# FishYuLi/BalancedGroupSoftmax

Measured on AMD Instinct MI355X. Metric: img/s fwd+bwd R50-FPN+BAGS 1333x800, 512 RoI (BASELINE metric: img/s/GPU fwd+bwd R50-FPN+BAGS 1333x800, 512 RoI; GroupSoftmax us/RoI), higher is better.
Workload: dtype f32 (conv/linear products on the bf16 MFMA from exact 3-way bf16 splits, fp32 accumulate: fp32-faithful)

## Files before the change

balancedgroupsoftmax_amd/backbone.py:

```python
import contextlib

import torch
import torch.nn as nn

from . import functional as BF
from .ops import OFFSET_PITCH, DeformConv
from .registry import BACKBONES, NECKS


def _trainable(*modules):
    return torch.is_grad_enabled() and any(
        p.requires_grad for m in modules if m is not None for p in m.parameters())


def _fold_conv_bn(conv, bn, pad_cin_to=None):
    w = conv.weight
    cbias = getattr(conv, 'bias', None)
    if w.is_cuda:
        ctx = contextlib.nullcontext() if _trainable(conv, bn) else torch.no_grad()
        with ctx:
            if bn is not None:
                return BF.fold_conv_bn(w, cbias, bn.weight, bn.bias, bn.running_mean,
                                       bn.running_var, bn.eps, cin_padded=pad_cin_to)
            return BF.fold_conv_bn(w, cbias, cin_padded=pad_cin_to)
# ... 124 lines not shown
    def _build_fold(self):
        f = dict(c1=_fold_conv_bn(self.conv1, self.bn1), c2=_fold_conv_bn(self.conv2, self.bn2),
                 c3=_fold_conv_bn(self.conv3, self.bn3))
        if self.downsample is not None:
            f['ds'] = _fold_conv_bn(self.downsample[0], self.downsample[1])
        if self.with_dcn:
            ow, ob = _fold_conv_bn(self.conv2_offset, None)
            padc = OFFSET_PITCH - ow.shape[0]
            f['off'] = (torch.nn.functional.pad(ow, (0, 0, 0, 0, 0, 0, 0, padc)).contiguous(),
                        torch.nn.functional.pad(ob, (0, padc)).contiguous())
        return f

    def run_bf16_storage(self, x, f):
        if self.with_dcn:
            raise NotImplementedError('Bottleneck.run_bf16_storage: a dcn block has no bf16-storage kernel '
                                      '(the deformable conv is fp32 only)')
        identity, fk = x, None
        if 'ds' in f:
            if x.is_cuda and BF.shortcut_fork_enabled():
                with BF.forked(x.device) as fk:
                    identity = BF.conv2d_nhwc(x, f['ds'][0], f['ds'][1], stride=self.stride)
            else:
                identity = BF.conv2d_nhwc(x, f['ds'][0], f['ds'][1], stride=self.stride)
        out = BF.conv2d_nhwc(x, f['c1'][0], f['c1'][1], relu=True)
        if self.groups > 1:
            out = BF.grouped_conv3x3_nhwc(out, f['c2'][0], f['c2'][1], self.groups, stride=self.stride,
                                          relu=True)
        else:
            out = BF.conv2d_nhwc(out, f['c2'][0], f['c2'][1], stride=self.stride, pad=1, relu=True)
        if fk is not None:
            fk.join()
        return BF.conv2d_nhwc(out, f['c3'][0], f['c3'][1], relu=True, residual=identity)

    def run(self, x, f):
        if x.dtype == torch.bfloat16:
            return self.run_bf16_storage(x, f)
        tagged = bool(getattr(x, '_bgs_consumers_mask', False))
        fuse = BF.fork_fusion_enabled() and torch.is_grad_enabled() and x.requires_grad
        if tagged and not fuse:
            raise RuntimeError("Bottleneck.run: x is a relu='consumers' block output but fork fusion is off")
        out_relu = 'consumers' if BF.fork_fusion_enabled() else True
        xin = x
        identity = x
        fk = None
        if 'ds' in f and not fuse and x.is_cuda and BF.shortcut_fork_enabled() and \
                not (torch.is_grad_enabled() and any(t.requires_grad for t in f['ds'] if t is not None)):
            with BF.forked(x.device) as fk:
                identity = BF.conv2d_nhwc(x, f['ds'][0], f['ds'][1], stride=self.stride)
        elif 'ds' in f:
            if fuse:
                identity, xin = BF.conv2d_autograd(x, f['ds'][0], f['ds'][1], stride=self.stride,
                                                   mask_input=tagged, passthrough=True)
            else:
                identity = BF.conv2d_autograd(x, f['ds'][0], f['ds'][1], stride=self.stride)
        first_pt = fuse and 'ds' not in f
        first_mask = tagged and 'ds' not in f
        if self.groups > 1 or self.with_dcn:
            out = BF.conv2d_autograd(xin, f['c1'][0], f['c1'][1], relu=True, mask_input=first_mask,
                                     passthrough=first_pt)
            if first_pt:
                out, identity = out
            if self.with_dcn:
                off = BF.conv2d_autograd(out, f['off'][0], f['off'][1], stride=self.stride, pad=1)
                out = BF.deform_conv3x3_nhwc(out, off, f['c2'][0], f['c2'][1], self.dcn_groups,
                                             stride=self.stride, relu=True)
            else:
                out = BF.grouped_conv3x3_nhwc(out, f['c2'][0], f['c2'][1], self.groups,
                                              stride=self.stride, relu=True)
            if fk is not None:
                fk.join()
            return BF.conv2d_autograd(out, f['c3'][0], f['c3'][1], relu=out_relu, residual=identity)
        out = BF.conv2d_autograd(xin, f['c1'][0], f['c1'][1], relu='consumers', mask_input=first_mask,
                                 passthrough=first_pt)
        if first_pt:
            out, identity = out
        if not fuse and BF.fused_c3_eligible(out, f['c2'][0], f['c3'][0], self.stride, identity):
            if fk is not None:
                fk.join()
            return BF.conv3x3_c3_fused_nhwc(out, f['c2'][0], f['c2'][1], f['c3'][0], f['c3'][1], residual=identity,
                                            relu3=True)
        out = BF.conv2d_autograd(out, f['c2'][0], f['c2'][1], stride=self.stride, pad=1,
                                 relu='consumers', mask_input=True)
        if fk is not None:
            fk.join()
        return BF.conv2d_autograd(out, f['c3'][0], f['c3'][1], relu=out_relu, residual=identity,
                                  mask_input=True)


@BACKBONES.register_module
class ResNet(nn.Module):
    arch_settings = {50: (3, 4, 6, 3), 101: (3, 4, 23, 3), 152: (3, 8, 36, 3)}

    def __init__(self, depth, num_stages=4, strides=(1, 2, 2, 2), dilations=(1, 1, 1, 1),
                 out_indices=(0, 1, 2, 3), style='pytorch', frozen_stages=-1, conv_cfg=None,
                 norm_cfg=dict(type='BN', requires_grad=True), norm_eval=True, dcn=None,
                 stage_with_dcn=(False, False, False, False), gcb=None,
                 stage_with_gcb=(False, False, False, False), gen_attention=None,
                 stage_with_gen_attention=((), (), (), ()), with_cp=False,
                 zero_init_residual=True, groups=1, base_width=4):
        super().__init__()
        if depth not in self.arch_settings:
            raise KeyError('invalid depth {} for resnet (bottleneck depths only)'.format(depth))
        if dcn:
            raise NotImplementedError('dcn (deformable convolution, gs_htc_dconv_* config) has no '
                                      'kernel in this build')
        if style != 'pytorch' or tuple(dilations) != (1, 1, 1, 1) or gcb or gen_attention:
            raise NotImplementedError('only the plain pytorch-style trunk of the BAGS configs')
        if norm_cfg.get('type', 'BN') != 'BN' or not norm_eval:
            raise NotImplementedError('BatchNorm in eval mode only (norm_eval=True is what every '
                                      'BAGS config uses); it is folded into the convs')
        self.depth, self.num_stages = depth, num_stages
# ... 46 lines not shown
        elif pretrained is not None:
            raise TypeError('pretrained must be a str or None')
        for m in self.modules():
            if isinstance(m, nn.Conv2d):
                nn.init.kaiming_normal_(m.weight, mode='fan_out', nonlinearity='relu')
            elif isinstance(m, nn.BatchNorm2d):
                nn.init.constant_(m.weight, 1)
                nn.init.constant_(m.bias, 0)
        for m in self.modules():
            if isinstance(m, Bottleneck):
                nn.init.constant_(m.bn3.weight, 0)
                if hasattr(m, 'conv2_offset'):
                    nn.init.constant_(m.conv2_offset.weight, 0)
                    nn.init.constant_(m.conv2_offset.bias, 0)

    def _build_stem(self):
        return _fold_conv_bn(self.conv1, self.bn1, pad_cin_to=4)

    @staticmethod
    def to_nhwc4(img):
        if img.is_cuda and not (torch.is_grad_enabled() and img.requires_grad):
            return BF.nchw_to_nhwc4(img)
        x = img.float().permute(0, 2, 3, 1)
        return torch.nn.functional.pad(x, (0, 4 - x.shape[3])).contiguous()

    def forward(self, img):
        return self.forward_partial(img, -1, len(self.res_layers) - 1)[1]

    def forward_partial(self, x, first, last, outs=()):
        outs = list(outs)
        if first < 0:
            x = self._forward_stem(x)
            first = 0
        for i in range(first, last + 1):
            for blk in getattr(self, self.res_layers[i]):
                x = blk.run(x, blk.folded())
            if i in self.out_indices:
                outs.append(BF.relu_gate(x))
        return x, tuple(outs)

    def _forward_stem(self, img):
        stem = self._cache.get((self.conv1, self.bn1), self._build_stem)
        frozen_stem = not (torch.is_grad_enabled() and (img.requires_grad or stem[0].requires_grad or
                                                        stem[1].requires_grad))
        if img.is_cuda and frozen_stem and img.shape[1] == 3 and tuple(stem[0].shape[:3]) == (64, 7, 7) \
                and BF.stem_fused_enabled():
            ws = self._stem_split.get((self.conv1, self.bn1),
                                      lambda: BF.stem_fused_split_weights(stem[0].detach()))
            x = BF.stem_fused(img, ws, stem[1].detach())
        else:
            x = self.to_nhwc4(img)
            x = BF.conv2d_autograd(x, stem[0], stem[1], stride=2, pad=3, relu=True)
            storage = (BF.bf16_storage_active() and not x.requires_grad and
                       not _trainable(*[getattr(self, n) for n in self.res_layers]))
            x = BF.maxpool3x3s2_nhwc(x, out_dtype=torch.bfloat16 if storage else torch.float32)
        return x

    def train(self, mode=True):
        super().train(mode)
        self._freeze_stages()
        if mode and self.norm_eval:
            for m in self.modules():
                if isinstance(m, nn.BatchNorm2d):
                    m.eval()
        return self


@BACKBONES.register_module
class ResNeXt(ResNet):
# ... 75 lines not shown
```

balancedgroupsoftmax_amd/capi.py:

```python
import ctypes
import os

_PKG = os.path.dirname(os.path.abspath(__file__))

c_i64p = ctypes.c_void_p
c_f32p = ctypes.c_void_p
c_ptr = ctypes.c_void_p

BGS_OK = 0
BGS_MAX_BINS = 16


class BgsLibraryError(RuntimeError):
    pass


class BgsCallError(RuntimeError):
    def __init__(self, fn, code, text):
        super().__init__('%s failed with code %d: %s' % (fn, code, text))
        self.code = code


SIGNATURES = {
    'bgs_version': (ctypes.c_int, []),
# ... 42 lines not shown
                            + [c_ptr]),
    'bgs_conv2d_workspace_bytes': (ctypes.c_size_t, [ctypes.c_longlong, ctypes.c_int]),
    'bgs_conv2d_nhwc_f32_ws': (ctypes.c_int, [c_f32p, c_f32p, c_f32p, c_f32p, c_f32p]
                               + [ctypes.c_int] * 11 + [c_ptr, ctypes.c_size_t, c_ptr]),
    'bgs_conv2d_dgrad_nhwc_f32_ws': (ctypes.c_int, [c_f32p, c_f32p, c_f32p, c_f32p, c_f32p]
                                     + [ctypes.c_int] * 10 + [c_ptr, ctypes.c_size_t, c_ptr]),
    'bgs_conv2d_dgrad_nhwc_f32': (ctypes.c_int, [c_f32p, c_f32p, c_f32p, c_f32p, c_f32p]
                                  + [ctypes.c_int] * 10 + [c_ptr]),
    'bgs_conv2d_wgrad_workspace_bytes': (ctypes.c_size_t, [ctypes.c_int] * 9),
    'bgs_conv2d_wgrad_nhwc_f32': (ctypes.c_int, [c_f32p, c_f32p, c_f32p, c_f32p]
                                  + [ctypes.c_int] * 10 + [c_ptr, c_ptr]),
    'bgs_fold_conv_bn_fwd': (ctypes.c_int, [c_f32p] * 6 + [ctypes.c_float] + [ctypes.c_int] * 5
                             + [c_f32p, c_f32p, c_ptr]),
    'bgs_fold_conv_bn_bwd': (ctypes.c_int, [c_f32p] * 7 + [ctypes.c_float] + [ctypes.c_int] * 5
                             + [c_f32p] * 4 + [c_ptr]),
    'bgs_conv2d_wgrad_bfx_workspace_bytes': (ctypes.c_size_t, [ctypes.c_int] * 9),
    'bgs_conv2d_wgrad_nhwc_f32_bfx': (ctypes.c_int, [c_f32p, c_f32p, c_f32p, c_f32p]
                                      + [ctypes.c_int] * 11 + [c_ptr, c_ptr]),
    'bgs_conv2d_wgrad_bfx_enable': (None, [ctypes.c_int]),
    'bgs_conv3x3_halo_nhwc_f32': (ctypes.c_int, [c_f32p, c_f32p, c_f32p, c_f32p] + [ctypes.c_int] * 6
                                  + [c_ptr]),
    'bgs_conv_bfx_weight_bytes': (ctypes.c_size_t, [ctypes.c_int, ctypes.c_int]),
    'bgs_conv_bfx_split_weights': (ctypes.c_int, [c_f32p, c_ptr, ctypes.c_int, ctypes.c_int, c_ptr]),
    'bgs_conv_dgrad_parity_enable': (None, [ctypes.c_int]),
    'bgs_conv_bfx_split_weights_dgrad': (ctypes.c_int, [c_f32p, c_ptr] + [ctypes.c_int] * 4 + [c_ptr]),
    'bgs_conv_bfx_workspace_bytes': (ctypes.c_size_t, [ctypes.c_longlong, ctypes.c_int, ctypes.c_int]),
    'bgs_conv2d_nhwc_f32_bfx_ws': (ctypes.c_int, [c_f32p, c_ptr, c_f32p, c_f32p, c_f32p]
                                   + [ctypes.c_int] * 12 + [c_ptr, ctypes.c_size_t, c_ptr]),
    'bgs_conv2d_dgrad_nhwc_f32_bfx_ws': (ctypes.c_int, [c_f32p, c_ptr, c_f32p, c_f32p, c_f32p]
                                         + [ctypes.c_int] * 11 + [c_ptr, ctypes.c_size_t, c_ptr]),
    'bgs_conv3x3_halo_bfx_workspace_bytes': (ctypes.c_size_t, [ctypes.c_int] * 5),
    'bgs_conv3x3_c3_fused_nhwc_f32_bfx': (ctypes.c_int, [c_f32p, c_ptr, c_f32p, c_ptr, c_f32p, c_f32p, c_f32p]
                                          + [ctypes.c_int] * 6 + [c_ptr]),
    'bgs_conv3x3_halo_nhwc_f32_bfx': (ctypes.c_int, [c_f32p, c_ptr, c_f32p, c_f32p]
                                      + [ctypes.c_int] * 7 + [c_ptr, ctypes.c_size_t, c_ptr]),
    'bgs_conv3x3_halo_nhwc_f32_bfx_ex': (ctypes.c_int, [c_f32p, c_ptr, c_f32p, c_f32p, c_f32p]
                                         + [ctypes.c_int] * 7 + [c_ptr, ctypes.c_size_t, c_ptr]),
    'bgs_conv3x3_planes_head_nhwc_f32_bfx': (ctypes.c_int, [c_f32p, c_ptr, c_f32p, c_ptr, c_f32p, c_f32p]
                                             + [ctypes.c_int] * 7 + [c_ptr]),
    'bgs_conv3x3_planes_head_eligible': (ctypes.c_int, [ctypes.c_int] * 6),
    'bgs_gs_loss_tuning': (None, [ctypes.c_int]),
    'bgs_gs_head_fold': (None, [ctypes.c_int]),
    'bgs_gs_loss_wavepriv_min_rows': (None, [ctypes.c_int]),
    'bgs_gs_merge_tuning': (None, [ctypes.c_int, ctypes.c_int]),
    'bgs_conv_bfx_wide_tuning': (None, [ctypes.c_int] * 3),
    'bgs_conv_bfx_wide_last_launch': (ctypes.c_int, []),
    'bgs_conv1x1_planes_enable': (None, [ctypes.c_int]),
    'bgs_conv1x1_planes_last_launch': (ctypes.c_int, []),
    'bgs_conv3x3_planes_enable': (None, [ctypes.c_int]),
    'bgs_conv3x3_planes_last_launch': (ctypes.c_int, []),
    'bgs_conv1x1_bres_enable': (None, [ctypes.c_int]),
    'bgs_conv1x1_bres_last_launch': (ctypes.c_int, []),
    'bgs_launch_census': (ctypes.c_int, [ctypes.c_int, ctypes.c_int]),
    'bgs_conv_bfx_tuning': (None, [ctypes.c_int] * 2),
    'bgs_conv_bfx_last_launch': (ctypes.c_int, [c_ptr, c_ptr]),
    'bgs_conv_tuning': (None, [ctypes.c_int] * 4),
    'bgs_conv_last_launch': (ctypes.c_int, [c_ptr, c_ptr, c_ptr, c_ptr]),
    'bgs_conv3x3_halo_bfx_tuning': (None, [ctypes.c_int] * 2),
    'bgs_conv3x3_halo_bfx_last_launch': (ctypes.c_int, [c_ptr, c_ptr]),
    'bgs_conv3x3_halo_bfx_last_wide': (ctypes.c_int, [c_ptr, c_ptr]),
    'bgs_conv3x3_halo_bfx_wide': (ctypes.c_int, [ctypes.c_int]),
    'bgs_grouped_conv3x3_nhwc_f32': (ctypes.c_int, [c_f32p, c_f32p, c_f32p, c_f32p] + [ctypes.c_int] * 7
                                     + [c_ptr]),
    'bgs_grouped_conv3x3_nhwc_bf16ops': (ctypes.c_int, [c_f32p, c_f32p, c_f32p, c_f32p] + [ctypes.c_int] * 7
                                         + [c_ptr]),
    'bgs_grouped_conv3x3_dgrad_nhwc_f32': (ctypes.c_int, [c_f32p, c_f32p, c_f32p] + [ctypes.c_int] * 6
# ... 225 lines not shown
```

balancedgroupsoftmax_amd/csrc/bottleneck_tail_planes.hip:

```cpp
#include <stdlib.h>

#include "conv_args.h"
#include "bfx_split.h"

using namespace bgs_conv;

namespace {

typedef __bf16 bf16x2 __attribute__((ext_vector_type(2)));
typedef __bf16 bf16x8 __attribute__((ext_vector_type(8)));
typedef unsigned u32x2 __attribute__((ext_vector_type(2)));
typedef unsigned u32x4 __attribute__((ext_vector_type(4)));

__device__ __forceinline__ unsigned pk_bf16(float a, float b) {
  const bf16x2 h = __builtin_convertvector(f32x2{a, b}, bf16x2);
  return __builtin_bit_cast(unsigned, h);
}

__device__ __forceinline__ void split3p(const f32x4 v, u32x2& hi, u32x2& mid, u32x2& lo) {
  hi = u32x2{pk_bf16(v[0], v[1]), pk_bf16(v[2], v[3])};
  const f32x4 r = {bfx_resid_lo(hi[0], v[0]), bfx_resid_hi(hi[0], v[1]), bfx_resid_lo(hi[1], v[2]),
                   bfx_resid_hi(hi[1], v[3])};
  mid = u32x2{pk_bf16(r[0], r[1]), pk_bf16(r[2], r[3])};
  const f32x4 r2 = {bfx_resid_lo(mid[0], r[0]), bfx_resid_hi(mid[0], r[1]), bfx_resid_lo(mid[1], r[2]),
                    bfx_resid_hi(mid[1], r[3])};
  lo = u32x2{pk_bf16(r2[0], r2[1]), pk_bf16(r2[2], r2[3])};
}

struct TailArgs {
  const float* x;
  const __bf16* ws2;
  const float* bias2;
  const __bf16* ws3;
  const float* bias3;
  const float* res;
  float* y;
  int N, H, W, relu3;
  int tiles_y, tiles_x, tiles, chunk;
};

constexpr int kOob = 0x7f000000;

__global__ __launch_bounds__(kThreads, 3) void bottleneck_tail_planes_kernel(TailArgs g) {
  constexpr int NS = 3, CM = 64, CO3 = 256, KC2 = 36, KC3 = 4;
  constexpr int PW = 10, PS = 12, PSLOTS = PW * PS;
  constexpr int AQ = PW * PW * 16, AQT = (AQ + kThreads - 1) / kThreads;
  constexpr int KS = PSLOTS * 32, PL = 4 * KS;
  constexpr int LDS_BYTES = NS * PL;
  constexpr int LD2 = CM + 4, S2_BYTES = 64 * LD2 * 4;
  constexpr int Y_OFF = 18 * 1024;
  constexpr int P3_CH = 64 * 32, P3_PL = KC3 * P3_CH;
  constexpr int LD4 = CO3 + 8;
  static_assert(S2_BYTES <= Y_OFF && Y_OFF + NS * P3_PL <= LDS_BYTES && 32 * LD4 * 4 <= LDS_BYTES, "overlays");
  __shared__ __attribute__((aligned(1024))) unsigned char lds[LDS_BYTES];

  const int tid = threadIdx.x, lane = tid & 63;
  const int wave = bgs::uniform(tid >> 6);
  const int wm = wave >> 1, wn = wave & 1;
  const int frow = lane & 31, fk = lane >> 5;
  const int vtile = (int)((blockIdx.x & 7) * g.chunk + (blockIdx.x >> 3));
  if (vtile >= g.tiles) return;
  const int per_img = g.tiles_y * g.tiles_x;
  const int n = vtile / per_img, trem = vtile - n * per_img;
  const int ty = trem / g.tiles_x, tx = trem - ty * g.tiles_x;
  const int h0 = ty * 8 - 1, w0 = tx * 8 - 1;

  const __amdgpu_buffer_rsrc_t x_rsrc = __builtin_amdgcn_make_buffer_rsrc(
      const_cast<float*>(g.x), 0, (int)((size_t)g.N * g.H * g.W * CM * 4), 0x00020000);
  f32x4 ra[AQT];
  int a_dst[AQT];
#pragma unroll
  for (int i = 0; i < AQT; ++i) {
    const int q = tid + kThreads * i;
    const bool use = q < AQ;
    const int pix = use ? q >> 4 : 0, kq = q & 15;
    const int ppy = pix / PW, ppx = pix - ppy * PW;
    const int hi = h0 + ppy, wi = w0 + ppx;
    const bool in = use && hi >= 0 && hi < g.H && wi >= 0 && wi < g.W;
    const int off = in ? (((n * g.H + hi) * g.W + wi) * CM + kq * 4) * 4 : kOob;
    ra[i] = __builtin_bit_cast(f32x4, __builtin_amdgcn_raw_buffer_load_b128(x_rsrc, off, 0, 0));
    const int quad = kq & 3;
// ... 112 lines not shown
#pragma unroll
  for (int kc = 0; kc < KC3; ++kc) {
    if (kc + 1 < KC3) {
      if (kc & 1) load_b3(kc + 1, f3a);
      else load_b3(kc + 1, f3b);
    }
    __builtin_amdgcn_sched_barrier(0);
    const bf16x8 (&fb3)[NS][2] = (kc & 1) ? f3b : f3a;
    bf16x8 fa3[NS][2];
#pragma unroll
    for (int s = 0; s < NS; ++s)
#pragma unroll
      for (int a = 0; a < 2; ++a) fa3[s][a] = *reinterpret_cast<const bf16x8*>(lds + a3_frag[a] + kc * P3_CH + s * P3_PL);
#pragma unroll
    for (int tt = NS - 1; tt >= 0; --tt)
#pragma unroll
      for (int i = 0; i <= tt; ++i)
#pragma unroll
        for (int a = 0; a < 2; ++a)
#pragma unroll
          for (int b = 0; b < 2; ++b)
            acc3[a][b] = __builtin_amdgcn_mfma_f32_32x32x16_bf16(fa3[i][a], fb3[tt - i][b], acc3[a][b], 0, 0, 0);
    __builtin_amdgcn_sched_barrier(0);
  }
  __syncthreads();

  const int e4 = (tid & 63) * 4, er0 = tid >> 6;
  f32x4 bias3 = {0.f, 0.f, 0.f, 0.f};
  if (g.bias3) bias3 = *reinterpret_cast<const f32x4*>(g.bias3 + e4);
  const int out_bytes = (int)((size_t)g.N * g.H * g.W * CO3 * 4);
  const __amdgpu_buffer_rsrc_t res_rsrc = __builtin_amdgcn_make_buffer_rsrc(
      const_cast<float*>(g.res ? g.res : g.x), 0, g.res ? out_bytes : 0, 0x00020000);
  const __amdgpu_buffer_rsrc_t y_rsrc = __builtin_amdgcn_make_buffer_rsrc(g.y, 0, out_bytes, 0x00020000);
#pragma unroll
  for (int a = 0; a < 2; ++a) {
    f32x4 rs[8];
#pragma unroll
    for (int ps = 0; ps < 8; ++ps) {
      const int m = a * 32 + er0 + ps * 4;
      const int ho = min(ty * 8 + (m >> 3), g.H - 1), wo = min(tx * 8 + (m & 7), g.W - 1);
      rs[ps] = __builtin_bit_cast(f32x4, __builtin_amdgcn_raw_buffer_load_b128(res_rsrc, (((n * g.H + ho) * g.W + wo) * CO3 + e4) * 4, 0, 0));
    }
#pragma unroll
    for (int b = 0; b < 2; ++b)
#pragma unroll
      for (int r = 0; r < 16; ++r) {
        const int i = (r & 3) + 8 * (r >> 2) + 4 * (lane >> 5);
        scratch[i * LD4 + wave * 64 + b * 32 + (lane & 31)] = acc3[a][b][r];
      }
    __syncthreads();
#pragma unroll
    for (int ps = 0; ps < 8; ++ps) {
      const int i = er0 + ps * 4;
      const int m = a * 32 + i;
      const int ho = ty * 8 + (m >> 3), wo = tx * 8 + (m & 7);
      f32x4 v = *reinterpret_cast<const f32x4*>(scratch + i * LD4 + e4);
      v += bias3;
      v += rs[ps];
      if (g.relu3) {
#pragma unroll
        for (int t = 0; t < 4; ++t) v[t] = fmaxf(v[t], 0.f);
      }
      if (ho < g.H && wo < g.W)
        __builtin_amdgcn_raw_buffer_store_b128(__builtin_bit_cast(u32x4, v), y_rsrc, (((n * g.H + ho) * g.W + wo) * CO3 + e4) * 4, 0, 0);
    }
    __syncthreads();
  }
}

}

int bgs_internal_bottleneck_tail_planes(const float* x, const void* w2split, const float* bias2, const void* w3split,
                                        const float* bias3, const float* residual, float* y, int N, int H, int W,
                                        int relu3, hipStream_t st) {
  const long long lim = kOob;
  if ((long long)N * H * W * 256 * 4 >= lim) return -1;
  TailArgs g;
  g.x = x;
  g.ws2 = reinterpret_cast<const __bf16*>(w2split);
  g.bias2 = bias2;
  g.ws3 = reinterpret_cast<const __bf16*>(w3split);
  g.bias3 = bias3;
  g.res = residual;
  g.y = y;
  g.N = N; g.H = H; g.W = W; g.relu3 = relu3;
  g.tiles_y = (H + 7) / 8;
  g.tiles_x = (W + 7) / 8;
  g.tiles = N * g.tiles_y * g.tiles_x;
  g.chunk = (g.tiles + 7) / 8;
  hipLaunchKernelGGL(bottleneck_tail_planes_kernel, dim3((unsigned)(8 * g.chunk)), dim3(kThreads), 0, st, g);
  return hipGetLastError() == hipSuccess ? BGS_OK : BGS_ERR_LAUNCH;
}
```

balancedgroupsoftmax_amd/functional.py:

```python
import ctypes
import itertools
import os

import torch

from . import capi

_WS = {}


def _workspace(nbytes, device):
    key = (device.index, capi.raw_stream(device))
    buf = _WS.get(key)
    if buf is None or buf.numel() < nbytes:
        buf = torch.empty(max(int(nbytes), 1 << 20), dtype=torch.uint8, device=device)
        _WS[key] = buf
    return buf


def reset_workspaces():
    _WS.clear()


_SIDE = {}
# ... 726 lines not shown
    capi.check('bgs_conv_bfx_split_weights_dgrad', rc)
    if cacheable:
        if key not in _SPLIT_CACHE and len(_SPLIT_CACHE) >= _SPLIT_CACHE_MAX:
            _SPLIT_CACHE.pop(next(iter(_SPLIT_CACHE)))
        _SPLIT_CACHE[key] = (w_krsc._version, (Cout, R, S, Cin), w_krsc, out, CacheFence(w_krsc.device))
    return out


def conv_bfx_tuning(tile=0, splitk=-1, halo_splits=-1, halo_variant=0, halo_geom=-1, halo_flags=0, halo_wide=-1):
    lib = capi.load()
    lib.bgs_conv_bfx_tuning(int(tile), int(splitk))
    lib.bgs_conv3x3_halo_bfx_tuning(int(halo_splits), int(halo_variant) | ((int(halo_geom) + 1) << 16) |
                                    (int(halo_flags) << 20) | ((int(halo_wide) + 1) << 24))


def set_halo_wide(mode):
    return capi.load().bgs_conv3x3_halo_bfx_wide(int(mode))


def conv_bfx_last_launch():
    import ctypes
    lib = capi.load()
    a, c, d, e, f, g = (ctypes.c_int() for _ in range(6))
    lib.bgs_conv_bfx_last_launch(ctypes.byref(a), ctypes.byref(c))
    lib.bgs_conv3x3_halo_bfx_last_launch(ctypes.byref(d), ctypes.byref(e))
    lib.bgs_conv3x3_halo_bfx_last_wide(ctypes.byref(f), ctypes.byref(g))
    return dict(tile=a.value & ~0x400, ring_stages=3 if a.value & 0x400 else 4, splits=c.value,
                halo_nb=d.value & 0xff, halo_variant=(d.value >> 8) & 0xff, halo_geom=d.value >> 16,
                halo_splits=e.value, halo_wide_units=f.value, halo_tail_units=g.value)


CENSUS = dict(bf16_ring8=0, grouped_lds=1, halo_bfx4=2, dma_ring64=3, gs_head_fused=4, conv1x1_bres=5,
              wgrad_bfx=6, roi_bwd_gather=7, bf16s=8, grouped_bf16s=9, bfx_wide=10, gs_scale_grad=11, halo_wide=12, stem_fused=13, fused_c3=14,
              planes_3x3=15, planes_1x1=16, planes_3x3_head=17)


def launch_census(reset=False):
    lib = capi.load()
    out = {k: lib.bgs_launch_census(v, 0) for k, v in CENSUS.items()}
    if reset:
        lib.bgs_launch_census(0, 1)
    return out


def conv_tuning(tile=0, bk=0, splitk=0, noswizzle=0):
    capi.load().bgs_conv_tuning(int(tile), int(bk), int(splitk), int(noswizzle))


def conv_last_launch():
    import ctypes
    a, b, c, d = (ctypes.c_int() for _ in range(4))
    capi.load().bgs_conv_last_launch(ctypes.byref(a), ctypes.byref(b), ctypes.byref(c), ctypes.byref(d))
    return dict(tile=a.value, bk=b.value, up=c.value, splits=d.value)


def _use_halo_bfx(M, Cout):
    env = os.environ.get('BGS_CONV_HALO')
    if env == '1':
        return True
    if env == '0':
        return False
    return M >= 2000


def _use_halo_kernel(M, Cout):
    env = os.environ.get('BGS_CONV_HALO')
    if env == '1':
# ... 11 lines not shown
    _FUSED_C3[0] = bool(on)
    return prev


def fused_c3_eligible(x, w2, w3, stride, residual):
    env = os.environ.get('BGS_FUSED_C3')
    on = _FUSED_C3[0] if env is None else env != '0'
    return (on and _CONV_MATH[0] == 'bf16x6' and x.is_cuda and x.dtype == torch.float32 and stride == 1
            and tuple(w2.shape[:3]) == (64, 3, 3) and w2.shape[3] == 64 and tuple(w3.shape) == (256, 1, 1, 64)
            and x.shape[3] == 64 and _use_halo_bfx(x.shape[0] * x.shape[1] * x.shape[2], 64)
            and x.shape[0] * ((x.shape[1] + 7) // 8) * ((x.shape[2] + 15) // 16) >= 700
            and not (torch.is_grad_enabled() and (x.requires_grad or w2.requires_grad or w3.requires_grad or
                                                  (residual is not None and residual.requires_grad))))


def conv3x3_c3_fused_nhwc(x, w2_krsc, bias2, w3_krsc, bias3, residual=None, relu3=True, out=None):
    _require_cuda(x, w2_krsc, bias2, w3_krsc, bias3, residual)
    lib = capi.load()
    assert x.dtype == torch.float32 and x.is_contiguous() and x.dim() == 4
    N, H, W, Cmid = x.shape
    Cout3 = w3_krsc.shape[0]
    assert tuple(w2_krsc.shape) == (Cmid, 3, 3, Cmid) and tuple(w3_krsc.shape) == (Cout3, 1, 1, Cmid)
    if residual is not None:
        assert tuple(residual.shape) == (N, H, W, Cout3) and residual.is_contiguous() and residual.dtype == torch.float32
    if out is None:
        out = torch.empty((N, H, W, Cout3), dtype=torch.float32, device=x.device)
    w2s = bfx_split_weights(w2_krsc.view(Cmid, 9 * Cmid), cache=True)
    w3s = bfx_split_weights(w3_krsc.view(Cout3, Cmid), cache=True)
    rc = lib.bgs_conv3x3_c3_fused_nhwc_f32_bfx(capi.ptr(x), capi.ptr(w2s), capi.ptr(bias2), capi.ptr(w3s),
                                               capi.ptr(bias3), capi.ptr(residual), capi.ptr(out), N, H, W, Cmid,
                                               Cout3, int(bool(relu3)), capi.current_stream(x.device))
    capi.check('bgs_conv3x3_c3_fused_nhwc_f32_bfx', rc)
    return out


def rpn_head_fusion_eligible(x, w_conv, w_head):
    if os.environ.get('BGS_RPN_HEAD_FUSION', '1') == '0' or _CONV_MATH[0] != 'bf16x6':
        return False
    if not x.is_cuda or x.dtype != torch.float32 or x.dim() != 4 or w_conv.dim() != 4 or w_head.dim() != 4:
        return False
    N, H, W, Cin = x.shape
    if tuple(w_conv.shape[1:]) != (3, 3, Cin) or tuple(w_head.shape[1:]) != (1, 1, w_conv.shape[0]):
        return False
    if not _use_halo_bfx(N * H * W, w_conv.shape[0]):
        return False
    return bool(capi.load().bgs_conv3x3_planes_head_eligible(N, H, W, Cin, w_conv.shape[0], w_head.shape[0]))


def conv3x3_head_fused_nhwc(x, w_krsc, bias, hw_krsc, hbias, relu=True):
    _require_cuda(x, w_krsc, bias, hw_krsc, hbias)
    lib = capi.load()
    assert x.dtype == torch.float32 and x.is_contiguous() and x.dim() == 4
    N, H, W, Cin = x.shape
    Cout, Ch = w_krsc.shape[0], hw_krsc.shape[0]
    assert tuple(w_krsc.shape) == (Cout, 3, 3, Cin) and tuple(hw_krsc.shape) == (Ch, 1, 1, Cout)
    assert w_krsc.is_contiguous() and hw_krsc.is_contiguous()
    ws = bfx_split_weights(w_krsc.view(Cout, 9 * Cin), cache=True)
    hs = bfx_split_weights(hw_krsc.view(Ch, Cout), cache=True)
    out = torch.empty((N, H, W, Ch), dtype=torch.float32, device=x.device)
    rc = lib.bgs_conv3x3_planes_head_nhwc_f32_bfx(capi.ptr(x), capi.ptr(ws), capi.ptr(bias), capi.ptr(hs),
                                                  capi.ptr(hbias), capi.ptr(out), N, H, W, Cin, Cout,
                                                  int(bool(relu)), Ch, capi.current_stream(x.device))
    capi.check('bgs_conv3x3_planes_head_nhwc_f32_bfx', rc)
    return out


# ... 1846 lines not shown
```

include/bgs.h:

```cpp
#ifndef BGS_H_
#define BGS_H_

#include <stddef.h>
#include <stdint.h>

#ifdef __cplusplus
extern "C" {
#endif

#define BGS_OK 0
#define BGS_ERR_INVALID_ARG 1
#define BGS_ERR_UNSUPPORTED 2
#define BGS_ERR_LAUNCH 3

#define BGS_MAX_BINS 16

typedef void* bgs_stream_t;

int bgs_version(void);
const char* bgs_error_string(int code);



int bgs_gs_prepare(const int64_t* labels, const int64_t* label2binlabel,
// ... 88 lines not shown
                         float* dgamma, float* dbeta, bgs_stream_t stream);


int bgs_conv3x3_halo_nhwc_f32(const float* x, const float* w, const float* bias, float* y, int N,
                              int H, int W, int Cin, int Cout, int relu, bgs_stream_t stream);

size_t bgs_conv_bfx_weight_bytes(int rows, int K);
int bgs_conv_bfx_split_weights(const float* w, void* out, int rows, int K, bgs_stream_t stream);
int bgs_conv_bfx_split_weights_dgrad(const float* w, void* out, int Cout, int R, int S, int Cin,
                                     bgs_stream_t stream);
size_t bgs_conv_bfx_workspace_bytes(long long M, int Cout, int K);
int bgs_conv2d_nhwc_f32_bfx_ws(const float* x, const void* wsplit, const float* bias,
                               const float* residual, float* y, int N, int H, int W, int Cin,
                               int Cout, int R, int S, int stride, int pad, int relu,
                               int residual_mode, int planes, void* workspace,
                               size_t workspace_bytes, bgs_stream_t stream);
int bgs_conv2d_dgrad_nhwc_f32_bfx_ws(const float* dy, const void* wt_split, const float* residual,
                                     const float* mask, float* dx, int N, int H, int W, int Cin,
                                     int Cout, int R, int S, int stride, int pad,
                                     int residual_mode, int planes, void* workspace,
                                     size_t workspace_bytes, bgs_stream_t stream);
size_t bgs_conv3x3_halo_bfx_workspace_bytes(int N, int H, int W, int Cin, int Cout);
int bgs_conv3x3_halo_nhwc_f32_bfx(const float* x, const void* wsplit, const float* bias, float* y,
                                  int N, int H, int W, int Cin, int Cout, int relu, int planes,
                                  void* workspace, size_t workspace_bytes, bgs_stream_t stream);
int bgs_conv3x3_halo_nhwc_f32_bfx_ex(const float* x, const void* wsplit, const float* bias,
                                     const float* mask, float* y, int N, int H, int W, int Cin,
                                     int Cout, int relu, int planes, void* workspace,
                                     size_t workspace_bytes, bgs_stream_t stream);
int bgs_conv3x3_c3_fused_nhwc_f32_bfx(const float* x, const void* w2split, const float* bias2,
                                      const void* w3split, const float* bias3, const float* residual,
                                      float* y, int N, int H, int W, int Cmid, int Cout3, int relu3,
                                      bgs_stream_t stream);
int bgs_conv3x3_planes_head_nhwc_f32_bfx(const float* x, const void* wsplit, const float* bias,
                                         const void* hsplit, const float* hbias, float* y, int N, int H,
                                         int W, int Cin, int Cout, int relu, int Chead, bgs_stream_t stream);
int bgs_conv3x3_planes_head_eligible(int N, int H, int W, int Cin, int Cout, int Chead);


int bgs_grouped_conv3x3_nhwc_f32(const float* x, const float* w, const float* bias, float* y,
                                 int N, int H, int W, int C, int groups, int stride, int relu,
                                 bgs_stream_t stream);

int bgs_grouped_conv3x3_nhwc_bf16ops(const float* x, const float* w, const float* bias, float* y,
                                     int N, int H, int W, int C, int groups, int stride, int relu,
                                     bgs_stream_t stream);

int bgs_conv2d_nhwc_bf16s(const void* x, const void* w_hi, const float* bias, const void* residual,
                          int residual_mode, int residual_bf16, void* y, int y_bf16, int N, int H, int W,
                          int Cin, int Cout, int R, int S, int stride, int pad, int relu,
                          bgs_stream_t stream);
int bgs_grouped_conv3x3_nhwc_bf16s(const void* x, const float* w, const float* bias, void* y, int N, int H,
                                   int W, int C, int groups, int stride, int relu, bgs_stream_t stream);
int bgs_maxpool3x3s2_nhwc_f32_to_bf16(const float* x, void* y, int N, int H, int W, int C,
                                      bgs_stream_t stream);

int bgs_grouped_conv3x3_dgrad_nhwc_f32(const float* dy, const float* wt, float* dx, int N, int H,
                                       int W, int C, int groups, int stride, bgs_stream_t stream);
size_t bgs_grouped_conv3x3_wgrad_workspace_bytes(int N, int H, int W, int C, int groups, int stride);
int bgs_grouped_conv3x3_wgrad_nhwc_f32(const float* x, const float* dy, float* dw, float* db, int N,
                                       int H, int W, int C, int groups, int stride, int accumulate,
                                       void* workspace, bgs_stream_t stream);

int bgs_deform_conv3x3_nhwc_f32(const float* x, const float* offset, const float* w, const float* bias,
                                float* y, int N, int H, int W, int C, int groups, int deformable_groups,
                                int off_pitch, int stride, int relu, bgs_stream_t stream);
// ... 248 lines not shown
```

include/bgs_tuning.h:

```cpp
#ifndef BGS_TUNING_H_
#define BGS_TUNING_H_

#include "bgs.h"

#ifdef __cplusplus
extern "C" {
#endif

int bgs_selftest_wave_reduce(const float* in, float* out, bgs_stream_t stream);
int bgs_selftest_mfma_peak(int blocks, int iters, float* out, bgs_stream_t stream);
int bgs_selftest_mfma_peak_bf16(int blocks, int iters, int random_operands, float* out, bgs_stream_t stream);

#define BGS_CENSUS_BF16_RING8 0
#define BGS_CENSUS_GROUPED_LDS 1
#define BGS_CENSUS_HALO_BFX4 2
#define BGS_CENSUS_DMA_RING64 3
#define BGS_CENSUS_GS_HEAD_FUSED 4
#define BGS_CENSUS_CONV1X1_BRES 5
#define BGS_CENSUS_WGRAD_BFX 6
#define BGS_CENSUS_ROI_BWD_GATHER 7
#define BGS_CENSUS_BF16S 8
#define BGS_CENSUS_GROUPED_BF16S 9
#define BGS_CENSUS_BFX_WIDE 10
#define BGS_CENSUS_GS_SCALE_GRAD 11
#define BGS_CENSUS_HALO_WIDE 12
#define BGS_CENSUS_STEM_FUSED 13
#define BGS_CENSUS_FUSED_C3 14
#define BGS_CENSUS_PLANES_3X3 15
#define BGS_CENSUS_PLANES_1X1 16
#define BGS_CENSUS_PLANES_3X3_HEAD 17
#define BGS_CENSUS_FAMILIES 20
int bgs_launch_census(int family, int reset);

void bgs_gs_head_debug_timestamps(unsigned long long* buf);
void bgs_gs_head_tuning(int rows_per_workgroup);
void bgs_gs_head_fold(int on);
void bgs_gs_head_variant(int variant);
int bgs_gs_head_variant_used(int N);

void bgs_conv_tuning(int tile, int bk, int splitk, int noswizzle);
int bgs_conv_last_launch(int* tile, int* bk, int* up, int* splits);
void bgs_conv_bfx_tuning(int tile, int splitk);
int bgs_conv_bfx_last_launch(int* tile, int* splits);
void bgs_conv3x3_halo_bfx_tuning(int splits, int variant);
int bgs_conv3x3_halo_bfx_last_launch(int* nb, int* splits);
int bgs_conv3x3_halo_bfx_last_wide(int* wide_units, int* tail_units);
int bgs_conv3x3_halo_bfx_wide(int mode);
void bgs_conv1x1_bres_enable(int on);
int bgs_conv1x1_bres_last_launch(void);
void bgs_conv_dgrad_parity_enable(int on);
void bgs_conv2d_wgrad_bfx_enable(int on);
void bgs_conv_bf16s_tuning(int variant);

void bgs_conv_bfx_wide_tuning(int mode, int nst, int splitk);
int bgs_conv_bfx_wide_last_launch(void);
void bgs_conv1x1_planes_enable(int mode);
int bgs_conv1x1_planes_last_launch(void);
void bgs_conv3x3_planes_enable(int mode);
int bgs_conv3x3_planes_last_launch(void);

void bgs_gs_loss_tuning(int prefetch);
void bgs_gs_loss_wavepriv_min_rows(int rows);
void bgs_gs_merge_tuning(int mode, int min_rows);
// ... 6 lines not shown
```

Measured before the change: 417.7.

## Fuse next bottleneck's conv1 into the conv3x3+conv1x1 tail kernel

Extends the fused bottleneck tail kernel with a templated variant. After writing the block output, that variant also computes the next block's 1x1 conv1 (64 or 128 output channels) plus bias and ReLU. It does this from register-resident output tiles, using 3-way bf16 split MFMA. The ResNet forward loop chains blocks so the precomputed conv1 output is passed into the next frozen fp32 block. This skips a separate launch and a re-read of the 256-channel activation. In exchange the tail kernel carries more registers and LDS, which may cost occupancy, and the fusion only applies to frozen width-64 blocks.

```diff
diff --git a/balancedgroupsoftmax_amd/backbone.py b/balancedgroupsoftmax_amd/backbone.py
--- a/balancedgroupsoftmax_amd/backbone.py
+++ b/balancedgroupsoftmax_amd/backbone.py
@@ -180,7 +180,10 @@
             fk.join()
         return BF.conv2d_nhwc(out, f['c3'][0], f['c3'][1], relu=True, residual=identity)
 
-    def run(self, x, f):
+    def run(self, x, f, next_c1=None, h=None):
+        if h is not None and (x.dtype == torch.bfloat16 or self.groups > 1 or self.with_dcn or
+                              (torch.is_grad_enabled() and x.requires_grad)):
+            raise RuntimeError('Bottleneck.run: a precomputed conv1 output is for the frozen fp32 block only')
         if x.dtype == torch.bfloat16:
             return self.run_bf16_storage(x, f)
         tagged = bool(getattr(x, '_bgs_consumers_mask', False))
@@ -218,13 +221,20 @@
             if fk is not None:
                 fk.join()
             return BF.conv2d_autograd(out, f['c3'][0], f['c3'][1], relu=out_relu, residual=identity)
-        out = BF.conv2d_autograd(xin, f['c1'][0], f['c1'][1], relu='consumers', mask_input=first_mask,
-                                 passthrough=first_pt)
-        if first_pt:
-            out, identity = out
+        if h is not None:
+            out = h
+        else:
+            out = BF.conv2d_autograd(xin, f['c1'][0], f['c1'][1], relu='consumers', mask_input=first_mask,
+                                     passthrough=first_pt)
+            if first_pt:
+                out, identity = out
         if not fuse and BF.fused_c3_eligible(out, f['c2'][0], f['c3'][0], self.stride, identity):
             if fk is not None:
                 fk.join()
+            if next_c1 is not None and BF.fused_c3_next_eligible(out, f['c2'][0], f['c3'][0], self.stride, identity,
+                                                                 next_c1[0], next_c1[1]):
+                return BF.conv3x3_c3_next_fused_nhwc(out, f['c2'][0], f['c2'][1], f['c3'][0], f['c3'][1], next_c1[0],
+                                                     next_c1[1], residual=identity, relu3=True)
             return BF.conv3x3_c3_fused_nhwc(out, f['c2'][0], f['c2'][1], f['c3'][0], f['c3'][1], residual=identity,
                                             relu3=True)
         out = BF.conv2d_autograd(out, f['c2'][0], f['c2'][1], stride=self.stride, pad=1,
@@ -337,9 +347,19 @@
         if first < 0:
             x = self._forward_stem(x)
             first = 0
-        for i in range(first, last + 1):
-            for blk in getattr(self, self.res_layers[i]):
-                x = blk.run(x, blk.folded())
+        chain = [(i, blk) for i in range(first, last + 1) for blk in getattr(self, self.res_layers[i])]
+        h, f = None, None
+        for k, (i, blk) in enumerate(chain):
+            nxt = chain[k + 1][1] if k + 1 < len(chain) else None
+            fn = None
+            if nxt is not None and blk.width == 64 and blk.stride == 1 and blk.groups == 1 and not blk.with_dcn \
+                    and nxt.groups == 1 and not nxt.with_dcn and not _trainable(nxt):
+                fn = nxt.folded()
+            r = blk.run(x, f if f is not None else blk.folded(), next_c1=None if fn is None else fn['c1'], h=h)
+            x, h = r if isinstance(r, tuple) else (r, None)
+            f = fn
+            if k + 1 < len(chain) and chain[k + 1][0] == i:
+                continue
             if i in self.out_indices:
                 outs.append(BF.relu_gate(x))
         return x, tuple(outs)
diff --git a/balancedgroupsoftmax_amd/capi.py b/balancedgroupsoftmax_amd/capi.py
--- a/balancedgroupsoftmax_amd/capi.py
+++ b/balancedgroupsoftmax_amd/capi.py
@@ -98,6 +98,10 @@
     'bgs_conv3x3_halo_bfx_workspace_bytes': (ctypes.c_size_t, [ctypes.c_int] * 5),
     'bgs_conv3x3_c3_fused_nhwc_f32_bfx': (ctypes.c_int, [c_f32p, c_ptr, c_f32p, c_ptr, c_f32p, c_f32p, c_f32p]
                                           + [ctypes.c_int] * 6 + [c_ptr]),
+    'bgs_conv3x3_c3_next_fused_nhwc_f32_bfx': (ctypes.c_int,
+                                               [c_f32p, c_ptr, c_f32p, c_ptr, c_f32p, c_f32p, c_f32p, c_ptr, c_f32p,
+                                                c_f32p] + [ctypes.c_int] * 7 + [c_ptr]),
+    'bgs_conv3x3_c3_next_eligible': (ctypes.c_int, [ctypes.c_int] * 6),
     'bgs_conv3x3_halo_nhwc_f32_bfx': (ctypes.c_int, [c_f32p, c_ptr, c_f32p, c_f32p]
                                       + [ctypes.c_int] * 7 + [c_ptr, ctypes.c_size_t, c_ptr]),
     'bgs_conv3x3_halo_nhwc_f32_bfx_ex': (ctypes.c_int, [c_f32p, c_ptr, c_f32p, c_f32p, c_f32p]
diff --git a/balancedgroupsoftmax_amd/csrc/bottleneck_tail_planes.hip b/balancedgroupsoftmax_amd/csrc/bottleneck_tail_planes.hip
--- a/balancedgroupsoftmax_amd/csrc/bottleneck_tail_planes.hip
+++ b/balancedgroupsoftmax_amd/csrc/bottleneck_tail_planes.hip
@@ -39,14 +39,31 @@
   int tiles_y, tiles_x, tiles, chunk;
 };
 
+struct TailNextArgs {
+  TailArgs t;
+  const __bf16* ws1n;
+  const float* bias1n;
+  float* h;
+};
+template <int NEXT> struct TailArgsOf { typedef TailNextArgs type; };
+template <> struct TailArgsOf<0> { typedef TailArgs type; };
+__device__ __forceinline__ const TailArgs& tail_base(const TailArgs& a) { return a; }
+__device__ __forceinline__ const TailArgs& tail_base(const TailNextArgs& a) { return a.t; }
+
 constexpr int kOob = 0x7f000000;
 
-__global__ __launch_bounds__(kThreads, 3) void bottleneck_tail_planes_kernel(TailArgs g) {
+template <int NEXT>
+__global__ __launch_bounds__(kThreads, 3) void bottleneck_tail_planes_kernel(typename TailArgsOf<NEXT>::type ga) {
+  static_assert(NEXT == 0 || NEXT == 64 || NEXT == 128, "width of the next block's conv1");
+  const TailArgs& g = tail_base(ga);
   constexpr int NS = 3, CM = 64, CO3 = 256, KC2 = 36, KC3 = 4;
   constexpr int PW = 10, PS = 12, PSLOTS = PW * PS;
   constexpr int AQ = PW * PW * 16, AQT = (AQ + kThreads - 1) / kThreads;
   constexpr int KS = PSLOTS * 32, PL = 4 * KS;
-  constexpr int LDS_BYTES = NS * PL;
+  constexpr int KCN = CO3 / 16, KCH = KCN / 2, KSN = 64 * 32 + 32, PLN = KCH * KSN;
+  constexpr int LDS_BYTES = NEXT ? NS * PLN : NS * PL;
+  static_assert(64 * (NEXT + 8) * 4 <= LDS_BYTES, "the h transpose tile overlays the planes");
+  static_assert(NS * PL <= LDS_BYTES && 3 * LDS_BYTES <= 160 * 1024, "three workgroups per CU");
   constexpr int LD2 = CM + 4, S2_BYTES = 64 * LD2 * 4;
   constexpr int Y_OFF = 18 * 1024;
   constexpr int P3_CH = 64 * 32, P3_PL = KC3 * P3_CH;
@@ -225,6 +242,7 @@
   const __amdgpu_buffer_rsrc_t res_rsrc = __builtin_amdgcn_make_buffer_rsrc(
       const_cast<float*>(g.res ? g.res : g.x), 0, g.res ? out_bytes : 0, 0x00020000);
   const __amdgpu_buffer_rsrc_t y_rsrc = __builtin_amdgcn_make_buffer_rsrc(g.y, 0, out_bytes, 0x00020000);
+  f32x4 vn[NEXT ? 2 : 1][NEXT ? 8 : 1];
 #pragma unroll
   for (int a = 0; a < 2; ++a) {
     f32x4 rs[8];
@@ -256,8 +274,113 @@
       }
       if (ho < g.H && wo < g.W)
         __builtin_amdgcn_raw_buffer_store_b128(__builtin_bit_cast(u32x4, v), y_rsrc, (((n * g.H + ho) * g.W + wo) * CO3 + e4) * 4, 0, 0);
+      if constexpr (NEXT > 0) vn[a][ps] = v;
     }
     __syncthreads();
+  }
+
+  if constexpr (NEXT > 0) {
+    constexpr int LDH = NEXT + 8, NA = NEXT == 128 ? 2 : 1;
+    const int a0 = NEXT == 128 ? 0 : (wave >> 1);
+    const int tn = NEXT == 128 ? wave : (wave & 1);
+    const __amdgpu_buffer_rsrc_t bn_rsrc = __builtin_amdgcn_make_buffer_rsrc(
+        const_cast<__bf16*>(ga.ws1n), 0, NS * KCN * NEXT * 32, 0x00020000);
+    const int bn_lane = ((tn * 32 + frow) * 16 + fk * 8) * 2;
+    auto load_bn = [&](int kc, bf16x8 (&dst)[NS]) {
+#pragma unroll
+      for (int s = 0; s < NS; ++s)
+        dst[s] = __builtin_bit_cast(bf16x8, __builtin_amdgcn_raw_buffer_load_b128(bn_rsrc, bn_lane, (s * KCN + kc) * NEXT * 32, 0));
+    };
+    bf16x8 fn[3][NS];
+    load_bn(0, fn[0]);
+    load_bn(1, fn[1]);
+    f32x4 vs[2][8];
+#pragma unroll
+    for (int ps = 0; ps < 8; ++ps) {
+      const u32x4 lo = __builtin_bit_cast(u32x4, vn[0][ps]), hi = __builtin_bit_cast(u32x4, vn[1][ps]);
+      u32x4 slo, shi;
+#pragma unroll
+      for (int t = 0; t < 4; ++t) {
+        const unsigned a0 = lo[t], a1 = hi[t];
+        const auto sw = __builtin_amdgcn_permlane32_swap(a0, a1, false, false);
+        slo[t] = sw[0];
+        shi[t] = sw[1];
+      }
+      vs[0][ps] = __builtin_bit_cast(f32x4, slo);
+      vs[1][ps] = __builtin_bit_cast(f32x4, shi);
+    }
+    const int kcl = (lane & 31) >> 2, kqn = lane & 3;
+    int an_frag[NA];
+#pragma unroll
+    for (int a = 0; a < NA; ++a) {
+      const int m = (a0 + a) * 32 + frow;
+      an_frag[a] = m * 32 + ((fk ^ ((m >> 3) & 1)) << 4);
+    }
+    f32x16 accn[NA];
+#pragma unroll
+    for (int a = 0; a < NA; ++a)
+#pragma unroll
+      for (int r = 0; r < 16; ++r) accn[a][r] = 0.f;
+#pragma unroll
+    for (int c = 0; c < 2; ++c) {
+#pragma unroll
+      for (int ps = 0; ps < 8; ++ps) {
+        const int i = (lane >> 5) * 32 + er0 + ps * 4;
+        u32x2 hh, mm, ll;
+        split3p(vs[c][ps], hh, mm, ll);
+        unsigned char* d = lds + kcl * KSN + i * 32 + (((kqn >> 1) ^ ((i >> 3) & 1)) << 4) + (kqn & 1) * 8;
+        *reinterpret_cast<u32x2*>(d) = hh;
+        *reinterpret_cast<u32x2*>(d + PLN) = mm;
+        *reinterpret_cast<u32x2*>(d + 2 * PLN) = ll;
+      }
+      __syncthreads();
+#pragma unroll
+      for (int k8 = 0; k8 < KCH; ++k8) {
+        const int kc = c * KCH + k8;
+        if (kc + 2 < KCN) load_bn(kc + 2, fn[(kc + 2) % 3]);
+        __builtin_amdgcn_sched_barrier(0);
+        const bf16x8 (&fbn)[NS] = fn[kc % 3];
+        bf16x8 fan[NS][NA];
+#pragma unroll
+        for (int s = 0; s < NS; ++s)
+#pragma unroll
+          for (int a = 0; a < NA; ++a) fan[s][a] = *reinterpret_cast<const bf16x8*>(lds + s * PLN + k8 * KSN + an_frag[a]);
+#pragma unroll
+        for (int tt = NS - 1; tt >= 0; --tt)
+#pragma unroll
+          for (int i = 0; i <= tt; ++i)
+#pragma unroll
+            for (int a = 0; a < NA; ++a)
+              accn[a] = __builtin_amdgcn_mfma_f32_32x32x16_bf16(fan[i][a], fbn[tt - i], accn[a], 0, 0, 0);
+        __builtin_amdgcn_sched_barrier(0);
+      }
+      __syncthreads();
+    }
+#pragma unroll
+    for (int a = 0; a < NA; ++a)
+#pragma unroll
+      for (int r = 0; r < 16; ++r) {
+        const int i = (a0 + a) * 32 + (r & 3) + 8 * (r >> 2) + 4 * (lane >> 5);
+        scratch[i * LDH + tn * 32 + (lane & 31)] = accn[a][r];
+      }
+    __syncthreads();
+    constexpr int TPRN = NEXT / 4, RPPN = kThreads / TPRN, EPN = 64 / RPPN;
+    const int n4 = (tid % TPRN) * 4, nr0 = tid / TPRN;
+    f32x4 biasn = {0.f, 0.f, 0.f, 0.f};
+    if (ga.bias1n) biasn = *reinterpret_cast<const f32x4*>(ga.bias1n + n4);
+    const __amdgpu_buffer_rsrc_t h_rsrc =
+        __builtin_amdgcn_make_buffer_rsrc(ga.h, 0, (int)((size_t)g.N * g.H * g.W * NEXT * 4), 0x00020000);
+#pragma unroll
+    for (int ps = 0; ps < EPN; ++ps) {
+      const int m = nr0 + ps * RPPN;
+      const int ho = ty * 8 + (m >> 3), wo = tx * 8 + (m & 7);
+      f32x4 v = *reinterpret_cast<const f32x4*>(scratch + m * LDH + n4);
+      v += biasn;
+#pragma unroll
+      for (int t = 0; t < 4; ++t) v[t] = fmaxf(v[t], 0.f);
+      if (ho < g.H && wo < g.W)
+        __builtin_amdgcn_raw_buffer_store_b128(__builtin_bit_cast(u32x4, v), h_rsrc, (((n * g.H + ho) * g.W + wo) * NEXT + n4) * 4, 0, 0);
+    }
   }
 }
 
@@ -281,6 +404,46 @@
   g.tiles_x = (W + 7) / 8;
   g.tiles = N * g.tiles_y * g.tiles_x;
   g.chunk = (g.tiles + 7) / 8;
-  hipLaunchKernelGGL(bottleneck_tail_planes_kernel, dim3((unsigned)(8 * g.chunk)), dim3(kThreads), 0, st, g);
+  hipLaunchKernelGGL(bottleneck_tail_planes_kernel<0>, dim3((unsigned)(8 * g.chunk)), dim3(kThreads), 0, st, g);
   return hipGetLastError() == hipSuccess ? BGS_OK : BGS_ERR_LAUNCH;
 }
+
+extern "C" int bgs_conv3x3_c3_next_eligible(int N, int H, int W, int Cmid, int Cout3, int Cnext) {
+  if (N <= 0 || H <= 0 || W <= 0 || Cmid != 64 || Cout3 != 256 || (Cnext != 64 && Cnext != 128)) return 0;
+  return (long long)N * H * W * 256 * 4 < (long long)kOob ? 1 : 0;
+}
+
+extern "C" int bgs_conv3x3_c3_next_fused_nhwc_f32_bfx(const float* x, const void* w2split, const float* bias2,
+                                                      const void* w3split, const float* bias3, const float* residual,
+                                                      float* y, const void* w1n_split, const float* bias1n, float* h,
+                                                      int N, int H, int W, int Cmid, int Cout3, int relu3, int Cnext,
+                                                      bgs_stream_t stream) {
+  if (N <= 0 || H <= 0 || W <= 0 || !x || !w2split || !w3split || !y || !w1n_split || !h) return BGS_ERR_INVALID_ARG;
+  if (!bgs_conv3x3_c3_next_eligible(N, H, W, Cmid, Cout3, Cnext)) return BGS_ERR_UNSUPPORTED;
+  if (((uintptr_t)x | (uintptr_t)w2split | (uintptr_t)w3split | (uintptr_t)y | (uintptr_t)residual | (uintptr_t)bias2 |
+       (uintptr_t)bias3 | (uintptr_t)w1n_split | (uintptr_t)bias1n | (uintptr_t)h) % 16 != 0)
+    return BGS_ERR_UNSUPPORTED;
+  TailNextArgs a;
+  TailArgs& g = a.t;
+  g.x = x;
+  g.ws2 = reinterpret_cast<const __bf16*>(w2split);
+  g.bias2 = bias2;
+  g.ws3 = reinterpret_cast<const __bf16*>(w3split);
+  g.bias3 = bias3;
+  g.res = residual;
+  g.y = y;
+  g.N = N; g.H = H; g.W = W; g.relu3 = relu3;
+  g.tiles_y = (H + 7) / 8;
+  g.tiles_x = (W + 7) / 8;
+  g.tiles = N * g.tiles_y * g.tiles_x;
+  g.chunk = (g.tiles + 7) / 8;
+  a.ws1n = reinterpret_cast<const __bf16*>(w1n_split);
+  a.bias1n = bias1n;
+  a.h = h;
+  const dim3 grid((unsigned)(8 * g.chunk)), block(kThreads);
+  if (Cnext == 64) hipLaunchKernelGGL(bottleneck_tail_planes_kernel<64>, grid, block, 0, (hipStream_t)stream, a);
+  else hipLaunchKernelGGL(bottleneck_tail_planes_kernel<128>, grid, block, 0, (hipStream_t)stream, a);
+  bgs_internal_census_bump(BGS_CENSUS_FUSED_C3);
+  bgs_internal_census_bump(BGS_CENSUS_FUSED_C3_NEXT);
+  return hipGetLastError() == hipSuccess ? BGS_OK : BGS_ERR_LAUNCH;
+}
diff --git a/balancedgroupsoftmax_amd/functional.py b/balancedgroupsoftmax_amd/functional.py
--- a/balancedgroupsoftmax_amd/functional.py
+++ b/balancedgroupsoftmax_amd/functional.py
@@ -782,7 +782,7 @@
 
 CENSUS = dict(bf16_ring8=0, grouped_lds=1, halo_bfx4=2, dma_ring64=3, gs_head_fused=4, conv1x1_bres=5,
               wgrad_bfx=6, roi_bwd_gather=7, bf16s=8, grouped_bf16s=9, bfx_wide=10, gs_scale_grad=11, halo_wide=12, stem_fused=13, fused_c3=14,
-              planes_3x3=15, planes_1x1=16, planes_3x3_head=17)
+              planes_3x3=15, planes_1x1=16, planes_3x3_head=17, fused_c3_next=18)
 
 
 def launch_census(reset=False):
@@ -860,6 +860,44 @@
                                                Cout3, int(bool(relu3)), capi.current_stream(x.device))
     capi.check('bgs_conv3x3_c3_fused_nhwc_f32_bfx', rc)
     return out
+
+
+def fused_c3_next_eligible(x, w2, w3, stride, residual, w1n, b1n=None, stride1n=1, pad1n=0):
+    if os.environ.get('BGS_TAIL_NEXT_C1', '1') == '0' or os.environ.get('BGS_FUSED_C3_PLANES', '1') == '0':
+        return False
+    if w1n is None or w1n.dim() != 4 or stride1n != 1 or pad1n != 0:
+        return False
+    if tuple(w1n.shape[1:]) != (1, 1, 256) or w1n.shape[0] not in (64, 128) or w1n.dtype != torch.float32:
+        return False
+    if torch.is_grad_enabled() and (w1n.requires_grad or (b1n is not None and b1n.requires_grad)):
+        return False
+    if not fused_c3_eligible(x, w2, w3, stride, residual):
+        return False
+    N, H, W, _ = x.shape
+    return bool(capi.load().bgs_conv3x3_c3_next_eligible(N, H, W, 64, 256, w1n.shape[0]))
+
+
+def conv3x3_c3_next_fused_nhwc(x, w2_krsc, bias2, w3_krsc, bias3, w1n_krsc, bias1n, residual=None, relu3=True):
+    _require_cuda(x, w2_krsc, bias2, w3_krsc, bias3, w1n_krsc, bias1n, residual)
+    lib = capi.load()
+    assert x.dtype == torch.float32 and x.is_contiguous() and x.dim() == 4
+    N, H, W, Cmid = x.shape
+    Cout3, Cnext = w3_krsc.shape[0], w1n_krsc.shape[0]
+    assert tuple(w2_krsc.shape) == (Cmid, 3, 3, Cmid) and tuple(w3_krsc.shape) == (Cout3, 1, 1, Cmid)
+    assert tuple(w1n_krsc.shape) == (Cnext, 1, 1, Cout3) and w1n_krsc.is_contiguous()
+    if residual is not None:
+        assert tuple(residual.shape) == (N, H, W, Cout3) and residual.is_contiguous() and residual.dtype == torch.float32
+    y = torch.empty((N, H, W, Cout3), dtype=torch.float32, device=x.device)
+    h = torch.empty((N, H, W, Cnext), dtype=torch.float32, device=x.device)
+    w2s = bfx_split_weights(w2_krsc.view(Cmid, 9 * Cmid), cache=True)
+    w3s = bfx_split_weights(w3_krsc.view(Cout3, Cmid), cache=True)
+    w1s = bfx_split_weights(w1n_krsc.view(Cnext, Cout3), cache=True)
+    rc = lib.bgs_conv3x3_c3_next_fused_nhwc_f32_bfx(capi.ptr(x), capi.ptr(w2s), capi.ptr(bias2), capi.ptr(w3s),
+                                                    capi.ptr(bias3), capi.ptr(residual), capi.ptr(y), capi.ptr(w1s),
+                                                    capi.ptr(bias1n), capi.ptr(h), N, H, W, Cmid, Cout3,
+                                                    int(bool(relu3)), Cnext, capi.current_stream(x.device))
+    capi.check('bgs_conv3x3_c3_next_fused_nhwc_f32_bfx', rc)
+    return y, h
 
 
 def rpn_head_fusion_eligible(x, w_conv, w_head):
diff --git a/include/bgs.h b/include/bgs.h
--- a/include/bgs.h
+++ b/include/bgs.h
@@ -144,6 +144,12 @@
                                       const void* w3split, const float* bias3, const float* residual,
                                       float* y, int N, int H, int W, int Cmid, int Cout3, int relu3,
                                       bgs_stream_t stream);
+int bgs_conv3x3_c3_next_fused_nhwc_f32_bfx(const float* x, const void* w2split, const float* bias2,
+                                           const void* w3split, const float* bias3, const float* residual,
+                                           float* y, const void* w1n_split, const float* bias1n, float* h,
+                                           int N, int H, int W, int Cmid, int Cout3, int relu3, int Cnext,
+                                           bgs_stream_t stream);
+int bgs_conv3x3_c3_next_eligible(int N, int H, int W, int Cmid, int Cout3, int Cnext);
 int bgs_conv3x3_planes_head_nhwc_f32_bfx(const float* x, const void* wsplit, const float* bias,
                                          const void* hsplit, const float* hbias, float* y, int N, int H,
                                          int W, int Cin, int Cout, int relu, int Chead, bgs_stream_t stream);
diff --git a/include/bgs_tuning.h b/include/bgs_tuning.h
--- a/include/bgs_tuning.h
+++ b/include/bgs_tuning.h
@@ -29,6 +29,7 @@
 #define BGS_CENSUS_PLANES_3X3 15
 #define BGS_CENSUS_PLANES_1X1 16
 #define BGS_CENSUS_PLANES_3X3_HEAD 17
+#define BGS_CENSUS_FUSED_C3_NEXT 18
 #define BGS_CENSUS_FAMILIES 20
 int bgs_launch_census(int family, int reset);
 
```

Measured after the change: 425.3, median of 6. 1.8% higher.
